# jjjkkyz/NU-NeRF

Measured on AMD Instinct MI355X. Metric: train rays/sec, higher is better.
Workload: dtype f32

## Files before the change

nu_nerf_amd/csrc/gemm_tn.hip:

```cpp
#include "gemm_epi.h"

__device__ unsigned long long nu_dbg_clk[2];

#define NU_TN_BATCH_MAX 16
struct NuGemmTNBatch {
    NuGemmTN p[NU_TN_BATCH_MAX];
    int blk0[NU_TN_BATCH_MAX + 1];
    int n, pad_;
};
static __device__ __forceinline__ int tn_batch_decode(const NuGemmTNBatch& b, int tile_edge, int& bx, int& split) {
    int pi = 0;
    for (int i = 1; i < b.n; ++i) pi = ((int)blockIdx.x >= b.blk0[i]) ? i : pi;
    const int tiles = ((b.p[pi].N1 + tile_edge - 1) / tile_edge) * ((b.p[pi].N2 + tile_edge - 1) / tile_edge);
    const int local = (int)blockIdx.x - b.blk0[pi];
    split = local / tiles;
    bx = local - split * tiles;
    return pi;
}

template <bool BIG, int PREC>
static __device__ __forceinline__ void tn_body(const NuGemmTN& g, const int bx, const int split, const int grp) {
    constexpr bool BF16 = PREC == 1;
    constexpr bool SPLIT = PREC == 2;
    constexpr int kPlane = 128 * NT_LDSH;
    __shared__ __attribute__((aligned(16))) float smem[SPLIT ? 1 : 2][SPLIT ? 3 * kPlane : 128 * NT_LDS];
    __bf16* const hA = reinterpret_cast<__bf16*>(&smem[0][0]);
    __bf16* const hB = hA + (SPLIT ? 3 : 1) * kPlane;

    const int tid = threadIdx.x;
    const int lane = tid & 63;
    const int wid = tid >> 6;
    const int wr = wid >> 1, wc = wid & 1;
    const int t2 = (g.N2 + 127) / 128;
    const int n1t = bx / t2, n2t = bx - n1t * t2;
    const int n1_0 = n1t * 128, n2_0 = n2t * 128;
    const int N1p = ((g.N1 + 127) / 128) * 128, N2p = t2 * 128;

    int rows_per = (g.P + g.S - 1) / g.S;
    rows_per = ((rows_per + TBK - 1) / TBK) * TBK;
    const int p_begin = split * rows_per;
    int p_end = p_begin + rows_per;
    p_end = p_end < g.P ? p_end : g.P;
    const int ntile = p_end > p_begin ? (p_end - p_begin + TBK - 1) / TBK : 0;
    const int npair = g.A1 ? 2 : 1;
    const int total = ntile * npair;

    const int c = tid & 127;
    const int kg = tid >> 7;
    const bool do_bias = (g.bias_slab != nullptr) && (n2t == 0);

    f32x16 acc[2][2];
#pragma unroll
    for (int i = 0; i < 2; ++i)
// ... 131 lines not shown
                acc[0][0] = __builtin_amdgcn_mfma_f32_32x32x16_bf16(a0, b0, acc[0][0], 0, 0, 0);
                acc[0][1] = __builtin_amdgcn_mfma_f32_32x32x16_bf16(a0, b1, acc[0][1], 0, 0, 0);
                acc[1][0] = __builtin_amdgcn_mfma_f32_32x32x16_bf16(a1, b0, acc[1][0], 0, 0, 0);
                acc[1][1] = __builtin_amdgcn_mfma_f32_32x32x16_bf16(a1, b1, acc[1][1], 0, 0, 0);
            }
        } else {
#pragma unroll
            for (int kk = 0; kk < 4; ++kk) {
                const float* As = &smem[0][0];
                const float* Bs = As + 128 * NT_LDS;
                const f32x4 a0 = *reinterpret_cast<const f32x4*>(&As[a_off + kk * 8]);
                const f32x4 a1 = *reinterpret_cast<const f32x4*>(&As[a_off + 32 * NT_LDS + kk * 8]);
                const f32x4 b0 = *reinterpret_cast<const f32x4*>(&Bs[b_off + kk * 8]);
                const f32x4 b1 = *reinterpret_cast<const f32x4*>(&Bs[b_off + 32 * NT_LDS + kk * 8]);
#pragma unroll
                for (int e = 0; e < 4; ++e) {
                    if (v00) acc[0][0] = __builtin_amdgcn_mfma_f32_32x32x2f32(a0[e], b0[e], acc[0][0], 0, 0, 0);
                    if (v01) acc[0][1] = __builtin_amdgcn_mfma_f32_32x32x2f32(a0[e], b1[e], acc[0][1], 0, 0, 0);
                    if (v10) acc[1][0] = __builtin_amdgcn_mfma_f32_32x32x2f32(a1[e], b0[e], acc[1][0], 0, 0, 0);
                    if (v11) acc[1][1] = __builtin_amdgcn_mfma_f32_32x32x2f32(a1[e], b1[e], acc[1][1], 0, 0, 0);
                }
            }
        }
        __syncthreads();
        if (t + 1 < total) {
            store_tile();
            __syncthreads();
        }
    }

    float* __restrict__ slab = g.slab + (long long)grp * g.sSlab + (long long)split * N1p * N2p;
#pragma unroll
    for (int tm = 0; tm < 2; ++tm)
#pragma unroll
        for (int tn = 0; tn < 2; ++tn) {
            const int col = n2_0 + wc * 64 + tn * 32 + li;
#pragma unroll
            for (int r = 0; r < 16; ++r) {
                const int row = n1_0 + wr * 64 + tm * 32 + (r & 3) + 8 * (r >> 2) + 4 * lh;
                slab[(long long)row * N2p + col] = acc[tm][tn][r];
            }
        }

    if (do_bias) {
        float* red = &smem[0][0];
        red[kg * 128 + c] = bs;
        __syncthreads();
        if (tid < 128) g.bias_slab[(long long)grp * g.sBiasSlab + (long long)split * N1p + n1_0 + tid] = red[tid] + red[128 + tid];
    }
}

template <bool BIG, int PREC>
__global__ __launch_bounds__(256, 2) void gemm_tn_kernel(NuGemmTN g) { tn_body<BIG, PREC>(g, blockIdx.x, blockIdx.y, blockIdx.z); }
template <bool BIG>
__global__ __launch_bounds__(256, 2) void gemm_tnb_kernel(NuGemmTNBatch b) {
    int bx, split;
    const int pi = tn_batch_decode(b, 128, bx, split);
    tn_body<BIG, 0>(b.p[pi], bx, split, 0);
}

#define TN16_ROWB 320
typedef short s16x4 __attribute__((ext_vector_type(4)));
typedef short s16x8 __attribute__((ext_vector_type(8)));

static __device__ __forceinline__ bf16x8 tn16_frag(const char* p) {
    const s16x4 lo = __builtin_amdgcn_ds_read_tr16_b64_v4i16((__attribute__((address_space(3))) s16x4*)(p));
    const s16x4 hi = __builtin_amdgcn_ds_read_tr16_b64_v4i16((__attribute__((address_space(3))) s16x4*)(p + 4 * TN16_ROWB));
    return __builtin_bit_cast(bf16x8, (s16x8)__builtin_shufflevector(lo, hi, 0, 1, 2, 3, 4, 5, 6, 7));
}

__global__ __launch_bounds__(256, 3) void gemm_tn16_kernel(NuGemmTN g) {
    __shared__ __attribute__((aligned(16))) char smem[2 * TBK * TN16_ROWB];
    char* const sA = smem;
    char* const sB = smem + TBK * TN16_ROWB;

    const int tid = threadIdx.x;
    const int lane = tid & 63;
    const int wid = tid >> 6;
    const int wr = wid >> 1, wc = wid & 1;
    const int t2 = (g.N2 + 127) / 128;
    const int n1t = blockIdx.x / t2, n2t = blockIdx.x - n1t * t2;
    const int split = blockIdx.y;
    const int n1_0 = n1t * 128, n2_0 = n2t * 128;
    const int grp = blockIdx.z;
    const int N1p = ((g.N1 + 127) / 128) * 128, N2p = t2 * 128;

    int rows_per = (g.P + g.S - 1) / g.S;
    rows_per = ((rows_per + TBK - 1) / TBK) * TBK;
    const int p_begin = split * rows_per;
    int p_end = p_begin + rows_per;
    p_end = p_end < g.P ? p_end : g.P;
    const int ntile = p_end > p_begin ? (p_end - p_begin + TBK - 1) / TBK : 0;
    const int npair = g.A1 ? 2 : 1;
    const int total = ntile * npair;

    const int cg = tid & 15;
    const int rr = tid >> 4;
    const bool do_bias = (g.bias_slab != nullptr) && (n2t == 0);

    f32x16 acc[2][2];
#pragma unroll
    for (int i = 0; i < 2; ++i)
#pragma unroll
        for (int j = 0; j < 2; ++j)
#pragma unroll
            for (int r = 0; r < 16; ++r) acc[i][j][r] = 0.0f;

    uint4 ra[2][2], rb[2][2];
    int nvalid = 0;
    bool pend_pair0 = true, pa16 = false, pb16 = false;
    float bs[8] = {0.f, 0.f, 0.f, 0.f, 0.f, 0.f, 0.f, 0.f};
    auto load_tile = [&](int t) {
// ... 229 lines not shown
    const int li = lane & 31, lh = lane >> 5;
    const int g4 = lane >> 4, tq = (lane & 15) >> 2, tc = lane & 3;
    const int a_off = (8 * (g4 >> 1) + tq) * TN16B_ROWB + (wr * 64 + 16 * (g4 & 1) + 4 * tc) * 2;
    const int b_off = (8 * (g4 >> 1) + tq) * TN16B_ROWB + (wc * 128 + 16 * (g4 & 1) + 4 * tc) * 2;
    for (int t = 0; t < total; ++t) {
        if (t + 1 < total) load_tile(t + 1);
#pragma unroll
        for (int ks = 0; ks < 2; ++ks) {
            const bf16x8 a0 = tn16b_frag(sA + a_off + ks * 16 * TN16B_ROWB);
            const bf16x8 a1 = tn16b_frag(sA + a_off + ks * 16 * TN16B_ROWB + 64);
            bf16x8 b[4];
#pragma unroll
            for (int tn = 0; tn < 4; ++tn) b[tn] = tn16b_frag(sB + b_off + ks * 16 * TN16B_ROWB + 64 * tn);
#pragma unroll
            for (int tn = 0; tn < 4; ++tn) {
                acc[0][tn] = __builtin_amdgcn_mfma_f32_32x32x16_bf16(a0, b[tn], acc[0][tn], 0, 0, 0);
                acc[1][tn] = __builtin_amdgcn_mfma_f32_32x32x16_bf16(a1, b[tn], acc[1][tn], 0, 0, 0);
            }
        }
        __syncthreads();
        if (t + 1 < total) {
            store_tile();
            __syncthreads();
        }
    }

    float* __restrict__ slab = g.slab + (long long)grp * g.sSlab + (long long)split * N1p * N2p;
#pragma unroll
    for (int tm = 0; tm < 2; ++tm)
#pragma unroll
        for (int tn = 0; tn < 4; ++tn) {
            const int col = n2_0 + wc * 128 + tn * 32 + li;
#pragma unroll
            for (int r = 0; r < 16; ++r) {
                const int row = n1_0 + wr * 64 + tm * 32 + (r & 3) + 8 * (r >> 2) + 4 * lh;
                slab[(long long)row * N2p + col] = acc[tm][tn][r];
            }
        }

    if (do_bias) {
        float* red = reinterpret_cast<float*>(smem);
#pragma unroll
        for (int e = 0; e < 8; ++e) red[rr * 256 + 8 * cg + e] = bs[e];
        __syncthreads();
        if (tid < 256) {
            float sum = 0.f;
#pragma unroll
            for (int r = 0; r < 16; ++r) sum += red[r * 256 + tid];
            g.bias_slab[(long long)grp * g.sBiasSlab + (long long)split * N1p + n1_0 + tid] = sum;
        }
    }
}


template <bool BIG>
static __device__ __forceinline__ void tn2_body(const NuGemmTN& g, const int bx, const int split, const int grp) {
    constexpr int T = 256;
    __shared__ __attribute__((aligned(16))) float smem[2][2][T * NT_LDS];
    const int tid = threadIdx.x;
    const int lane = tid & 63;
    const int wid = tid >> 6;
    const int wr = wid >> 1, wc = wid & 1;
    const int t2 = (g.N2 + T - 1) / T;
    const int n1t = bx / t2, n2t = bx - n1t * t2;
    const int n1_0 = n1t * T, n2_0 = n2t * T;
    const int N1p = ((g.N1 + 127) / 128) * 128, N2p = ((g.N2 + 127) / 128) * 128;

    int rows_per = (g.P + g.S - 1) / g.S;
    rows_per = ((rows_per + TBK - 1) / TBK) * TBK;
    const int p_begin = split * rows_per;
    int p_end = p_begin + rows_per;
    p_end = p_end < g.P ? p_end : g.P;
    const int ntile = p_end > p_begin ? (p_end - p_begin + TBK - 1) / TBK : 0;
    const int npair = g.A1 ? 2 : 1;
    const int total = ntile * npair;

    const int c = tid & (T - 1);
    const int kg = tid / T;
    const bool do_bias = (g.bias_slab != nullptr) && (n2t == 0);

    f32x16 acc[2][4];
#pragma unroll
    for (int i = 0; i < 2; ++i)
#pragma unroll
        for (int j = 0; j < 4; ++j)
#pragma unroll
            for (int r = 0; r < 16; ++r) acc[i][j][r] = 0.0f;

    f32x4 ra4[4], rb4[4];
    int nvalid = 16;
    bool pend_pair0 = true;
    float bs = 0.f;
    const char* __restrict__ ldA = nullptr;
    const char* __restrict__ ldB = nullptr;
    int ld_lda = 0, ld_ldb = 0, ld_ca = 0, ld_cb = 0, ld_pbase = 0, ld_pbase_u = 0;
    int nvalid_ld = 16;
    bool pair0_ld = true;
    auto load_begin = [&](int t) {
        const int pair = t >= ntile ? 1 : 0;
        const int kt = t - pair * ntile;
        ldA = (const char*)(pair ? g.A1 + (long long)grp * g.sA1 : g.A0 + (long long)grp * g.sA0);
        ldB = (const char*)(pair ? g.B1 + (long long)grp * g.sB1 : g.B0 + (long long)grp * g.sB0);
        ld_lda = pair ? g.lda1 : g.lda0;
        ld_ldb = pair ? g.ldb1 : g.ldb0;
        ld_ca = n1_0 + c; ld_cb = n2_0 + c;
        ld_ca = ld_ca < ld_lda ? ld_ca : ld_lda - 1;
        ld_cb = ld_cb < ld_ldb ? ld_cb : ld_ldb - 1;
        ld_pbase = p_begin + kt * TBK + kg * 16;
        ld_pbase_u = p_begin + kt * TBK;
        nvalid_ld = p_end - ld_pbase;
        pair0_ld = pair == 0;
    };
    auto load_piece = [&](int i, int e0, int e1) {
#pragma unroll
        for (int e = e0; e < e1; ++e) {
            int pr = ld_pbase + 4 * i + e;
            pr = pr < p_end ? pr : p_end - 1;
            if (BIG) {
                ra4[i][e] = reinterpret_cast<const float*>(ldA)[(long long)pr * ld_lda + ld_ca];
                rb4[i][e] = reinterpret_cast<const float*>(ldB)[(long long)pr * ld_ldb + ld_cb];
            } else {
                const unsigned oa = ((unsigned)pr * (unsigned)ld_lda + (unsigned)ld_ca) * 4u;
                const unsigned ob = ((unsigned)pr * (unsigned)ld_ldb + (unsigned)ld_cb) * 4u;
                ra4[i][e] = *reinterpret_cast<const float*>(ldA + oa);
                rb4[i][e] = *reinterpret_cast<const float*>(ldB + ob);
            }
        }
    };
    auto store_piece = [&](int st, int i) {
#pragma unroll
        for (int e = 0; e < 4; ++e) {
            const bool ok = 4 * i + e < nvalid;
            ra4[i][e] = ok ? ra4[i][e] : 0.f;
            rb4[i][e] = ok ? rb4[i][e] : 0.f;
        }
        if (do_bias && pend_pair0) bs += (ra4[i][0] + ra4[i][1]) + (ra4[i][2] + ra4[i][3]);
        *reinterpret_cast<f32x4*>(&smem[st][0][c * NT_LDS + kg * 16 + 4 * i]) = ra4[i];
        *reinterpret_cast<f32x4*>(&smem[st][1][c * NT_LDS + kg * 16 + 4 * i]) = rb4[i];
    };
    auto load_tile = [&](int t) {
        load_begin(t);
#pragma unroll
        for (int i = 0; i < 4; ++i) load_piece(i, 0, 4);
        nvalid = nvalid_ld; pend_pair0 = pair0_ld;
    };
    auto store_tile = [&](int st) {
#pragma unroll
        for (int i = 0; i < 4; ++i) store_piece(st, i);
    };

    if (total > 0) {
        load_tile(0);
        store_tile(0);
        if (total > 1) load_tile(1);
    }
    __syncthreads();

    const int li = lane & 31, lh = lane >> 5;
    const int a_off = (wr * 64 + li) * NT_LDS + 4 * lh;
    const int b_off = (wc * 128 + li) * NT_LDS + 4 * lh;
    struct FragT { f32x4 a[2]; f32x4 b[4]; };
    FragT F0, F1;
    const int kg_u = __builtin_amdgcn_readfirstlane(kg);
    const char* rpA = nullptr;
    const char* rpB = nullptr;
    int prA = 0, prB = 0;
    auto ld_rows_begin = [&]() {
        int pr = ld_pbase_u + kg_u * 16;
        pr = pr < p_end ? pr : p_end - 1;
        prA = prB = pr;
        rpA = ldA + (long long)pr * ld_lda * 4;
        rpB = ldB + (long long)pr * ld_ldb * 4;
    };
    auto ld_one = [&](bool isA, int i, int e) {
        if (isA) {
            ra4[i][e] = *reinterpret_cast<const float*>(rpA + (unsigned)ld_ca * 4u);
            const bool more = prA + 1 < p_end;
            rpA += more ? (long long)ld_lda * 4 : 0;
            prA += more ? 1 : 0;
        } else {
            rb4[i][e] = *reinterpret_cast<const float*>(rpB + (unsigned)ld_cb * 4u);
            const bool more = prB + 1 < p_end;
            rpB += more ? (long long)ld_ldb * 4 : 0;
            prB += more ? 1 : 0;
        }
    };
    auto st_zero = [&](bool isA, int i) {
#pragma unroll
        for (int e = 0; e < 4; ++e) {
            if (isA) ra4[i][e] = (4 * i + e < nvalid) ? ra4[i][e] : 0.f;
            else rb4[i][e] = (4 * i + e < nvalid) ? rb4[i][e] : 0.f;
        }
    };
    bool bias_on = false;
    auto st_write = [&](bool isA, int st, int i) {
        if (isA) {
            const float rs = (ra4[i][0] + ra4[i][1]) + (ra4[i][2] + ra4[i][3]);
            bs += bias_on ? rs : 0.f;
            *reinterpret_cast<f32x4*>(&smem[st][0][c * NT_LDS + kg * 16 + 4 * i]) = ra4[i];
        } else {
            *reinterpret_cast<f32x4*>(&smem[st][1][c * NT_LDS + kg * 16 + 4 * i]) = rb4[i];
        }
    };
    int cur = 0;
    if (total > 0) {
#pragma unroll
        for (int i = 0; i < 2; ++i) F0.a[i] = *reinterpret_cast<const f32x4*>(&smem[0][0][a_off + 32 * i * NT_LDS]);
#pragma unroll
        for (int j = 0; j < 4; ++j) F0.b[j] = *reinterpret_cast<const f32x4*>(&smem[0][1][b_off + 32 * j * NT_LDS]);
    }
#define TN_PIN __builtin_amdgcn_sched_barrier(0);
#define TN_M(F, e, i, j) acc[i][j] = __builtin_amdgcn_mfma_f32_32x32x2f32(F.a[i][e], F.b[j][e], acc[i][j], 0, 0, 0); TN_PIN
#define TN_SLOT(F, e, ...) TN_SLOT_(F, e, __VA_ARGS__)
#define TN_SLOT_(F, e, X0, X1, X2, X3, X4, X5, X6)                                                   \
    TN_M(F, e, 0, 0) X0; TN_PIN TN_M(F, e, 0, 1) X1; TN_PIN TN_M(F, e, 0, 2) X2; TN_PIN TN_M(F, e, 0, 3) X3; TN_PIN     \
    TN_M(F, e, 1, 0) X4; TN_PIN TN_M(F, e, 1, 1) X5; TN_PIN TN_M(F, e, 1, 2) X6; TN_PIN TN_M(F, e, 1, 3)
#define TN_RDA(F, ST, kk, i) F.a[i] = *reinterpret_cast<const f32x4*>(&smem[ST][0][a_off + 32 * (i) * NT_LDS + (kk) * 8])
#define TN_RDB(F, ST, kk, j) F.b[j] = *reinterpret_cast<const f32x4*>(&smem[ST][1][b_off + 32 * (j) * NT_LDS + (kk) * 8])
#define TN_READS(F, ST, kk) TN_RDA(F, ST, kk, 0), TN_RDA(F, ST, kk, 1), TN_RDB(F, ST, kk, 0), TN_RDB(F, ST, kk, 1), TN_RDB(F, ST, kk, 2), TN_RDB(F, ST, kk, 3), (void)0
#define TN_LD2(i, e) ld_one(true, i, e), ld_one(false, i, e), ld_one(true, i, (e) + 1), ld_one(false, i, (e) + 1), (void)0, (void)0, (void)0
#define TN_ST(i) st_zero(true, i), st_write(true, cur ^ 1, i), st_zero(false, i), st_write(false, cur ^ 1, i), (void)0, (void)0, (void)0
    for (int t = 0; t < total; ++t) {
        bias_on = do_bias && pend_pair0 && t + 1 < total;
        load_begin(t + 2 < total ? t + 2 : total - 1);
        ld_rows_begin();
        TN_SLOT(F0, 0, TN_ST(0))
        TN_SLOT(F0, 1, TN_LD2(0, 0))
        TN_SLOT(F0, 2, TN_LD2(0, 2))
        TN_SLOT(F0, 3, TN_READS(F1, cur, 1))
        TN_SLOT(F1, 0, TN_ST(1))
        TN_SLOT(F1, 1, TN_LD2(1, 0))
        TN_SLOT(F1, 2, TN_LD2(1, 2))
        TN_SLOT(F1, 3, TN_READS(F0, cur, 2))
        TN_SLOT(F0, 0, TN_ST(2))
        TN_SLOT(F0, 1, TN_ST(3))
        TN_SLOT(F0, 2, TN_LD2(2, 0))
        TN_SLOT(F0, 3, TN_READS(F1, cur, 3))
        __syncthreads();
        TN_SLOT(F1, 0, TN_LD2(2, 2))
        TN_SLOT(F1, 1, TN_LD2(3, 0))
        TN_SLOT(F1, 2, TN_LD2(3, 2))
        TN_SLOT(F1, 3, TN_READS(F0, cur ^ 1, 0))
        nvalid = nvalid_ld; pend_pair0 = pair0_ld;
        cur ^= 1;
    }
#undef TN_PIN
#undef TN_M
#undef TN_SLOT
#undef TN_SLOT_
#undef TN_RDA
#undef TN_RDB
#undef TN_READS
#undef TN_LD2
#undef TN_ST

    float* __restrict__ slab = g.slab + (long long)grp * g.sSlab + (long long)split * N1p * N2p;
#pragma unroll
    for (int tm = 0; tm < 2; ++tm)
#pragma unroll
        for (int tn = 0; tn < 4; ++tn) {
            const int col = n2_0 + wc * 128 + tn * 32 + li;
#pragma unroll
            for (int r = 0; r < 16; ++r) {
                const int row = n1_0 + wr * 64 + tm * 32 + (r & 3) + 8 * (r >> 2) + 4 * lh;
                slab[(long long)row * N2p + col] = acc[tm][tn][r];
            }
        }
    if (do_bias) {
        float* red = &smem[0][0][0];
        red[kg * T + c] = bs;
        __syncthreads();
        if (tid < T) g.bias_slab[(long long)grp * g.sBiasSlab + (long long)split * N1p + n1_0 + tid] = red[tid] + red[T + tid];
    }
}

template <bool BIG>
__global__ __launch_bounds__(512, 2) void gemm_tn2_kernel(NuGemmTN g) { tn2_body<BIG>(g, blockIdx.x, blockIdx.y, blockIdx.z); }
template <bool BIG>
__global__ __launch_bounds__(512, 2) void gemm_tn2b_kernel(NuGemmTNBatch b) {
    int bx, split;
    const int pi = tn_batch_decode(b, 256, bx, split);
    tn2_body<BIG>(b.p[pi], bx, split, 0);
}

static bool nu_tn_big_tile(int N1, int N2, int groups, int prec, int S) {
    if ((prec & 3) == 2 || (N1 % 256) != 0 || (N2 % 256) != 0) return false;
    return (long long)(N1 / 256) * (N2 / 256) * (groups > 0 ? groups : 1) * S >= 192;
}
extern "C" int nu_wgrad_pick_split(int P, int N1, int N2, int groups, int prec) {
    if (groups < 1) groups = 1;
    const int rows_min = P <= 8192 ? 128 : 256;
    const int cap = (P + rows_min - 1) / rows_min > 0 ? (P + rows_min - 1) / rows_min : 1;
    if ((N1 % 256) == 0 && (N2 % 256) == 0) {
        int S = 256 / ((N1 / 256) * (N2 / 256) * groups);
        if (S < 1) S = 1;
        if (S > cap) S = cap;
        if (nu_tn_big_tile(N1, N2, groups, prec, S)) return S;
    }
    int S = 512 / (nu_cdiv(N1, 128) * nu_cdiv(N2, 128) * groups);
    if (S < 1) S = 1;
    if (S > cap) S = cap;
    return S;
}

int nu_gemm_tn_launch(const NuGemmTN& g, hipStream_t stream) {
    if (g.N1 <= 0 || g.N2 <= 0 || g.S <= 0) return NU_ERR_ARG;
    if ((g.lda0 & 3) || (g.ldb0 & 3) || (g.A1 && ((g.lda1 & 3) || (g.ldb1 & 3)))) return NU_ERR_ARG;
    const int prec = g.bf16 & 3;
    if (prec == 3 || ((g.bf16 & ~3) && prec != 1)) return NU_ERR_ARG;
    const bool big_tile = nu_tn_big_tile(g.N1, g.N2, g.groups, g.bf16, g.S);
    const long long max_ld = (g.lda0 > g.ldb0 ? g.lda0 : g.ldb0) > (g.A1 ? (g.lda1 > g.ldb1 ? g.lda1 : g.ldb1) : 0)
                                 ? (g.lda0 > g.ldb0 ? g.lda0 : g.ldb0) : (g.lda1 > g.ldb1 ? g.lda1 : g.ldb1);
    const bool big = (long long)g.P * max_ld * 4 >= (1LL << 32);
    if (prec == 0 && big_tile) {
        dim3 grid2((g.N1 / 256) * (g.N2 / 256), g.S, g.groups > 0 ? g.groups : 1);
        if (big) hipLaunchKernelGGL((gemm_tn2_kernel<true>), grid2, dim3(512), 0, stream, g);
        else hipLaunchKernelGGL((gemm_tn2_kernel<false>), grid2, dim3(512), 0, stream, g);
        return nu_launch_status();
    }
    dim3 grid(nu_cdiv(g.N1, 128) * nu_cdiv(g.N2, 128), g.S, g.groups > 0 ? g.groups : 1), block(256);
    if (prec == 1) {
        auto ok = [](const float* p, int ld, bool h) { return p == nullptr || ((((uintptr_t)p) & 15) == 0 && ld >= 8 && (!h || (ld & 7) == 0)); };
        const bool vec = ok(g.A0, g.lda0, g.bf16 & NU_TN_A0_16) && ok(g.B0, g.ldb0, g.bf16 & NU_TN_B0_16) &&
                         ok(g.A1, g.lda1, g.bf16 & NU_TN_A1_16) && ok(g.B1, g.ldb1, g.bf16 & NU_TN_B1_16) &&
                         ((g.sA0 | g.sB0 | g.sA1 | g.sB1) & 7) == 0;
        if (vec) {
            if (big_tile) {
                dim3 grid2((g.N1 / 256) * (g.N2 / 256), g.S, g.groups > 0 ? g.groups : 1);
                hipLaunchKernelGGL(gemm_tn16x256_kernel, grid2, dim3(512), 0, stream, g);
            } else {
                hipLaunchKernelGGL(gemm_tn16_kernel, grid, block, 0, stream, g);
            }
            return nu_launch_status();
        }
    }
    if (big) {
        if (prec == 2) hipLaunchKernelGGL((gemm_tn_kernel<true, 2>), grid, block, 0, stream, g);
        else if (prec == 1) hipLaunchKernelGGL((gemm_tn_kernel<true, 1>), grid, block, 0, stream, g);
        else hipLaunchKernelGGL((gemm_tn_kernel<true, 0>), grid, block, 0, stream, g);
    } else {
        if (prec == 2) hipLaunchKernelGGL((gemm_tn_kernel<false, 2>), grid, block, 0, stream, g);
        else if (prec == 1) hipLaunchKernelGGL((gemm_tn_kernel<false, 1>), grid, block, 0, stream, g);
        else hipLaunchKernelGGL((gemm_tn_kernel<false, 0>), grid, block, 0, stream, g);
    }
    return nu_launch_status();
}

struct NuReduceBatch {
    NuReduceDesc d[NU_REDUCE_MAX];
    int n;
};

__global__ __launch_bounds__(256) void slab_reduce_batched_kernel(NuReduceBatch b) {
    __shared__ float red[256];
    int di = 0;
    for (int i = 1; i < b.n; ++i) di = ((int)blockIdx.x >= b.d[i].blk_begin) ? i : di;
    const float* __restrict__ slab = b.d[di].slab;
    float* __restrict__ out = b.d[di].out;
    const int S = b.d[di].S, N1 = b.d[di].N1, N2 = b.d[di].N2, rs = b.d[di].rs, G = b.d[di].G;
    const long long ss = b.d[di].ss;
    const int opb = 256 / G;
    const int o = threadIdx.x % opb, g = threadIdx.x / opb;
    const int idx = ((int)blockIdx.x - b.d[di].blk_begin) * opb + o;
    const bool live = idx < N1 * N2;
    float v = 0.f;
    int n1 = 0, n2 = 0;
    if (live) {
        n1 = idx / N2;
        n2 = idx - n1 * N2;
        const float* p = slab + (long long)n1 * rs + n2;
        float s0 = 0.f, s1 = 0.f, s2 = 0.f, s3 = 0.f;
        int s = g;
        for (; s + 3 * G < S; s += 4 * G) {
// ... 202 lines not shown
        float* bias_slab = w.db ? slab + slab_per * g.groups : nullptr;
        ws += (nu_wgrad_workspace_bytes(g.N1, g.N2, g.S, g.groups) + 255) / 256 * 64;
        for (int z = 0; z < g.groups; ++z) {
            NuGemmTN& q = b.p[np];
            q = g;
            q.groups = 1;
            q.A0 = g.A0 + z * g.sA0; q.B0 = g.B0 + z * g.sB0;
            q.A1 = g.A1 ? g.A1 + z * g.sA1 : nullptr; q.B1 = g.B1 ? g.B1 + z * g.sB1 : nullptr;
            q.slab = slab + z * slab_per; q.bias_slab = bias_slab ? bias_slab + z * bias_per : nullptr;
            q.sSlab = 0; q.sBiasSlab = 0;
            b.blk0[np++] = blocks;
            blocks += nu_cdiv(g.N1, edge) * nu_cdiv(g.N2, edge) * g.S;
            rc = nu_reduce_push(c->descs, &c->ndesc, c->cap, q.slab, g.S, g.N1, g.N2, N2p, (long long)N1p * N2p, w.dW + z * w.sW, w.ldw, 1.0f, 0);
            if (rc == NU_OK && w.db)
                rc = nu_reduce_push(c->descs, &c->ndesc, c->cap, q.bias_slab, g.S, g.N1, 1, 1, N1p, w.db + z * w.sDb, 1, 1.0f, 0);
            if (rc != NU_OK) return rc;
        }
        flops += w.flops; abytes += w.bytes;
    }
    b.blk0[np] = blocks;
    b.n = np; b.pad_ = 0;
    nu_ctx_ev_begin(c, stream);
    if (klass == 2) hipLaunchKernelGGL((gemm_tn2b_kernel<false>), dim3(blocks), dim3(512), 0, stream, b);
    else hipLaunchKernelGGL((gemm_tnb_kernel<false>), dim3(blocks), dim3(256), 0, stream, b);
    rc = nu_launch_status();
    nu_ctx_ev_end(c, stream, 1.0, flops, abytes);
    return rc;
}

static int wgrad_launch_single(NuOpCtx* c, NuWgradItem& w, hipStream_t stream) {
    NuGemmTN& g = w.g;
    g.S = nu_wgrad_pick_split(g.P, g.N1, g.N2, g.groups, g.bf16 & 3);
    float* ws;
    long long nb;
    int rc = nu_ctx_take(c, nu_wgrad_workspace_bytes(g.N1, g.N2, g.S, g.groups), 2 * g.groups, stream, &ws, &nb);
    if (rc != NU_OK) return rc;
    nu_ctx_ev_begin(c, stream);
    rc = nu_wgrad_enqueue(&g, w.dW, w.ldw, w.sW, w.db, w.sDb, ws, nb, c->descs, &c->ndesc, c->cap, stream);
    nu_ctx_ev_end(c, stream, 1.0, w.flops, w.bytes);
    return rc;
}

extern "C" int nu_wgrad_flush(NuOpCtx* c, hipStream_t stream) {
    const int n = c->npend;
    if (n <= 0 || c->pend == nullptr) return NU_OK;
    NuWgradItem* it = c->pend;
    c->npend = 0;
    int klass[NU_WGRAD_QUEUE_MAX];
    if (n > NU_WGRAD_QUEUE_MAX) return NU_ERR_ARG;
    int pmax = 0;
    for (int i = 0; i < n; ++i) {
        NuGemmTN& g = it[i].g;
        if (g.groups < 1) g.groups = 1;
        klass[i] = ((g.bf16 & 3) == 0 && (g.bf16 & ~3) == 0 && !tn_item_big(g) && g.groups <= NU_TN_BATCH_MAX) ? 1 : 0;
        if (klass[i] && g.P > pmax) pmax = g.P;
    }
    const int rows_min = pmax <= 8192 ? 128 : 256;
    auto plan = [&](int k, int edge, int target) -> long long {
        long long work = 0;
        for (int i = 0; i < n; ++i)
            if (klass[i] == k) work += (long long)it[i].g.P * nu_cdiv(it[i].g.N1, edge) * nu_cdiv(it[i].g.N2, edge) * it[i].g.groups;
        if (work == 0) return 0;
        long long rows = nu_cdivl(work, target);
        rows = rows < rows_min ? rows_min : rows;
        rows = nu_cdivl(rows, TBK) * TBK;
        while (true) {
            long long wgs = 0;
            for (int i = 0; i < n; ++i)
                if (klass[i] == k) wgs += nu_cdivl(it[i].g.P, rows) * nu_cdiv(it[i].g.N1, edge) * nu_cdiv(it[i].g.N2, edge) * it[i].g.groups;
            if (wgs <= target || rows >= (1LL << 30)) { for (int i = 0; i < n; ++i) if (klass[i] == k) it[i].g.S = (int)nu_cdivl(it[i].g.P, rows); return wgs; }
            rows += TBK;
        }
    };
    for (int i = 0; i < n; ++i)
        if (klass[i] == 1 && (it[i].g.N1 % 256) == 0 && (it[i].g.N2 % 256) == 0) klass[i] = 2;
    if (plan(2, 256, 256) < 192)
        for (int i = 0; i < n; ++i) if (klass[i] == 2) klass[i] = 1;
    plan(1, 128, 1024);
    for (int i = 0; i < n; ++i)
        if (klass[i] == 0) { const int rc = wgrad_launch_single(c, it[i], stream); if (rc != NU_OK) return rc; }
    for (int k = 2; k >= 1; --k) {
        int idx[NU_WGRAD_QUEUE_MAX], m = 0, nprob = 0;
        long long bytes = 0;
        for (int i = 0; i <= n; ++i) {
            const bool mine = i < n && klass[i] == k;
            long long need = 0;
            if (mine) need = (nu_wgrad_workspace_bytes(it[i].g.N1, it[i].g.N2, it[i].g.S, it[i].g.groups) + 255) / 256 * 256;
            const bool full = mine && m > 0 && (nprob + it[i].g.groups > NU_TN_BATCH_MAX || bytes + need > c->arena_floats * 4);
            if ((i == n || full) && m > 0) {
                const int rc = wgrad_launch_batch(c, it, idx, m, k, stream);
                if (rc != NU_OK) return rc;
                m = 0; nprob = 0; bytes = 0;
            }
            if (mine) { idx[m++] = i; nprob += it[i].g.groups; bytes += need; }
        }
    }
    return NU_OK;
}

extern "C" int nu_wgrad_defer(NuOpCtx* c, const NuGemmTN* g, float* dW, int ldw, long long sW, float* db, long long sDb, double flops,
                              double bytes, hipStream_t stream) {
    if (g->P <= 0) return NU_OK;
    NuWgradItem w;
    w.g = *g; w.dW = dW; w.ldw = ldw; w.pad_ = 0; w.sW = sW; w.db = db; w.sDb = sDb; w.flops = flops; w.bytes = bytes;
    if (w.g.groups < 1) w.g.groups = 1;
    if (c->pend == nullptr || c->pend_cap <= 0) return wgrad_launch_single(c, w, stream);
    if (c->npend >= c->pend_cap || c->npend >= NU_WGRAD_QUEUE_MAX) {
// ... 33 lines not shown
```

Before: 99590.

## Rewrite fp32 TN wgrad GEMM with row-major LDS tiles and vectorized loads

Replaces the tn2 body with a templated tnr_body (T=128 or 256). It stores operands row-major in LDS and loads 16-byte vectors from global memory instead of scalar column loads. A compile-time schedule interleaves LDS reads, global loads, stores and bias sums between single-k MFMA steps, and small edge tiles use fewer MFMAs. The 128-tile batched kernel and the single-launch fp32 path now route aligned inputs through this body. This is meant to cut global load count and LDS traffic, but it needs alignment checks and adds code size and register pressure.

```diff
diff --git a/nu_nerf_amd/csrc/gemm_tn.hip b/nu_nerf_amd/csrc/gemm_tn.hip
--- a/nu_nerf_amd/csrc/gemm_tn.hip
+++ b/nu_nerf_amd/csrc/gemm_tn.hip
@@ -1,4 +1,6 @@
 #include "gemm_epi.h"
+#include <type_traits>
+#include <utility>
 
 __device__ unsigned long long nu_dbg_clk[2];
 
@@ -236,12 +238,6 @@
 
 template <bool BIG, int PREC>
 __global__ __launch_bounds__(256, 2) void gemm_tn_kernel(NuGemmTN g) { tn_body<BIG, PREC>(g, blockIdx.x, blockIdx.y, blockIdx.z); }
-template <bool BIG>
-__global__ __launch_bounds__(256, 2) void gemm_tnb_kernel(NuGemmTNBatch b) {
-    int bx, split;
-    const int pi = tn_batch_decode(b, 128, bx, split);
-    tn_body<BIG, 0>(b.p[pi], bx, split, 0);
-}
 
 #define TN16_ROWB 320
 typedef short s16x4 __attribute__((ext_vector_type(4)));
@@ -577,15 +573,31 @@
     }
 }
 
-
-template <bool BIG>
-static __device__ __forceinline__ void tn2_body(const NuGemmTN& g, const int bx, const int split, const int grp) {
-    constexpr int T = 256;
-    __shared__ __attribute__((aligned(16))) float smem[2][2][T * NT_LDS];
+template <class F, int... I>
+static __device__ __forceinline__ void tn_static_for_(F&& f, std::integer_sequence<int, I...>) { (f(std::integral_constant<int, I>{}), ...); }
+template <int N, class F>
+static __device__ __forceinline__ void tn_static_for(F&& f) { tn_static_for_(f, std::make_integer_sequence<int, N>{}); }
+
+template <int T, bool BIAS>
+struct TnrSched {
+    static constexpr bool active(int s, int k) {
+        return k == 0 ? (BIAS && s <= 14) : k == 1 ? (BIAS && s == 14) : k == 2 ? true : k == 3 ? true : k == 4 ? T == 256 :
+               k == 5 ? s < 8 : k == 6 ? (s >= 1 && s <= 8) : (s == 14 || (BIAS && (s == 4 || s == 8 || s == 12 || s == 15)));
+    }
+    static constexpr int rank(int s, int k) { int n = 0; for (int i = 0; i < k; ++i) n += active(s, i) ? 1 : 0; return n; }
+    static constexpr int gap(int s, int k, int nm) { return rank(s, k) * nm / rank(s, 8); }
+};
+
+template <bool BIG, int T>
+static __device__ __forceinline__ void tnr_body(const NuGemmTN& g, const int bx, const int split, const int grp) {
+    constexpr int RS = T + 32;
+    constexpr int NB = T / 64;
+    constexpr int CG = T / 4;
+    constexpr int OPW = TBK * RS;
+    __shared__ __attribute__((aligned(16))) float smem[4 * OPW];
     const int tid = threadIdx.x;
     const int lane = tid & 63;
     const int wid = tid >> 6;
-    const int wr = wid >> 1, wc = wid & 1;
     const int t2 = (g.N2 + T - 1) / T;
     const int n1t = bx / t2, n2t = bx - n1t * t2;
     const int n1_0 = n1t * T, n2_0 = n2t * T;
@@ -600,199 +612,177 @@
     const int npair = g.A1 ? 2 : 1;
     const int total = ntile * npair;
 
-    const int c = tid & (T - 1);
+    const int cg = tid % CG;
+    const int r0 = tid / CG;
+    const int c = tid % T;
     const int kg = tid / T;
     const bool do_bias = (g.bias_slab != nullptr) && (n2t == 0);
 
-    f32x16 acc[2][4];
+    f32x16 acc[2][NB];
 #pragma unroll
     for (int i = 0; i < 2; ++i)
 #pragma unroll
-        for (int j = 0; j < 4; ++j)
+        for (int j = 0; j < NB; ++j)
 #pragma unroll
             for (int r = 0; r < 16; ++r) acc[i][j][r] = 0.0f;
 
-    f32x4 ra4[4], rb4[4];
-    int nvalid = 16;
-    bool pend_pair0 = true;
-    float bs = 0.f;
+    f32x4 ra[4], rb[4];
+    int nvalid = 0, nvalid_ld = 0;
     const char* __restrict__ ldA = nullptr;
     const char* __restrict__ ldB = nullptr;
-    int ld_lda = 0, ld_ldb = 0, ld_ca = 0, ld_cb = 0, ld_pbase = 0, ld_pbase_u = 0;
-    int nvalid_ld = 16;
-    bool pair0_ld = true;
-    auto load_begin = [&](int t) {
+    int ld_lda = 0, ld_ldb = 0, ld_ca = 0, ld_cb = 0, ld_pbase = 0;
+    const char* const pA0 = (const char*)(g.A0 + (long long)grp * g.sA0);
+    const char* const pB0 = (const char*)(g.B0 + (long long)grp * g.sB0);
+    const char* const pA1 = (const char*)(g.A1 + (long long)grp * g.sA1);
+    const char* const pB1 = (const char*)(g.B1 + (long long)grp * g.sB1);
+    const int lda0 = g.lda0, ldb0 = g.ldb0, lda1 = g.lda1, ldb1 = g.ldb1;
+    auto load_begin = [&](int t) __attribute__((always_inline)) {
         const int pair = t >= ntile ? 1 : 0;
         const int kt = t - pair * ntile;
-        ldA = (const char*)(pair ? g.A1 + (long long)grp * g.sA1 : g.A0 + (long long)grp * g.sA0);
-        ldB = (const char*)(pair ? g.B1 + (long long)grp * g.sB1 : g.B0 + (long long)grp * g.sB0);
-        ld_lda = pair ? g.lda1 : g.lda0;
-        ld_ldb = pair ? g.ldb1 : g.ldb0;
-        ld_ca = n1_0 + c; ld_cb = n2_0 + c;
-        ld_ca = ld_ca < ld_lda ? ld_ca : ld_lda - 1;
-        ld_cb = ld_cb < ld_ldb ? ld_cb : ld_ldb - 1;
-        ld_pbase = p_begin + kt * TBK + kg * 16;
-        ld_pbase_u = p_begin + kt * TBK;
+        ldA = pair ? pA1 : pA0;
+        ldB = pair ? pB1 : pB0;
+        ld_lda = pair ? lda1 : lda0;
+        ld_ldb = pair ? ldb1 : ldb0;
+        ld_ca = n1_0 + 4 * cg; ld_cb = n2_0 + 4 * cg;
+        ld_ca = ld_ca <= ld_lda - 4 ? ld_ca : ld_lda - 4;
+        ld_cb = ld_cb <= ld_ldb - 4 ? ld_cb : ld_ldb - 4;
+        ld_pbase = p_begin + kt * TBK;
         nvalid_ld = p_end - ld_pbase;
-        pair0_ld = pair == 0;
     };
-    auto load_piece = [&](int i, int e0, int e1) {
-#pragma unroll
-        for (int e = e0; e < e1; ++e) {
-            int pr = ld_pbase + 4 * i + e;
-            pr = pr < p_end ? pr : p_end - 1;
-            if (BIG) {
-                ra4[i][e] = reinterpret_cast<const float*>(ldA)[(long long)pr * ld_lda + ld_ca];
-                rb4[i][e] = reinterpret_cast<const float*>(ldB)[(long long)pr * ld_ldb + ld_cb];
-            } else {
-                const unsigned oa = ((unsigned)pr * (unsigned)ld_lda + (unsigned)ld_ca) * 4u;
-                const unsigned ob = ((unsigned)pr * (unsigned)ld_ldb + (unsigned)ld_cb) * 4u;
-                ra4[i][e] = *reinterpret_cast<const float*>(ldA + oa);
-                rb4[i][e] = *reinterpret_cast<const float*>(ldB + ob);
-            }
-        }
+    auto ld_one = [&](bool isA, int j) __attribute__((always_inline)) {
+        int pr = ld_pbase + r0 + 8 * j;
+        pr = pr < p_end ? pr : p_end - 1;
+        const char* base = isA ? ldA : ldB;
+        const int ld = isA ? ld_lda : ld_ldb, col = isA ? ld_ca : ld_cb;
+        f32x4 v;
+        if (BIG) v = *reinterpret_cast<const f32x4*>(base + ((long long)pr * ld + col) * 4);
+        else v = *reinterpret_cast<const f32x4*>(base + ((unsigned)pr * (unsigned)ld + (unsigned)col) * 4u);
+        if (isA) ra[j] = v; else rb[j] = v;
     };
-    auto store_piece = [&](int st, int i) {
-#pragma unroll
-        for (int e = 0; e < 4; ++e) {
-            const bool ok = 4 * i + e < nvalid;
-            ra4[i][e] = ok ? ra4[i][e] : 0.f;
-            rb4[i][e] = ok ? rb4[i][e] : 0.f;
-        }
-        if (do_bias && pend_pair0) bs += (ra4[i][0] + ra4[i][1]) + (ra4[i][2] + ra4[i][3]);
-        *reinterpret_cast<f32x4*>(&smem[st][0][c * NT_LDS + kg * 16 + 4 * i]) = ra4[i];
-        *reinterpret_cast<f32x4*>(&smem[st][1][c * NT_LDS + kg * 16 + 4 * i]) = rb4[i];
+    auto st_one = [&](bool isA, int st, int j) __attribute__((always_inline)) {
+        const bool ok = r0 + 8 * j < nvalid;
+        const f32x4 z = {0.f, 0.f, 0.f, 0.f};
+        const f32x4 v = isA ? ra[j] : rb[j];
+        *reinterpret_cast<f32x4*>(&smem[(2 * st + (isA ? 0 : 1)) * OPW + (r0 + 8 * j) * RS + 4 * cg]) = ok ? v : z;
     };
-    auto load_tile = [&](int t) {
-        load_begin(t);
-#pragma unroll
-        for (int i = 0; i < 4; ++i) load_piece(i, 0, 4);
-        nvalid = nvalid_ld; pend_pair0 = pair0_ld;
+
+    if (total > 0) {
+        load_begin(0);
+#pragma unroll
+        for (int j = 0; j < 4; ++j) { ld_one(true, j); ld_one(false, j); }
+        nvalid = nvalid_ld;
+#pragma unroll
+        for (int j = 0; j < 4; ++j) { st_one(true, 0, j); st_one(false, 0, j); }
+        if (total > 1) {
+            load_begin(1);
+#pragma unroll
+            for (int j = 0; j < 4; ++j) { ld_one(true, j); ld_one(false, j); }
+            nvalid = nvalid_ld;
+        }
+    }
+    __syncthreads();
+
+    const int wid_u = __builtin_amdgcn_readfirstlane(wid);
+    int arow = (wid_u >> 1) * 64, bcol = (wid_u & 1) * (T / 2), own_a = 2, own_b = NB, live_a = 2, live_b = NB;
+    if constexpr (T == 128) {
+        const int nlr = g.N1 - n1_0 >= 128 ? 4 : (g.N1 - n1_0 + 31) / 32, nlc = g.N2 - n2_0 >= 128 ? 4 : (g.N2 - n2_0 + 31) / 32;
+        if (nlc <= 2) { arow = 32 * wid_u; bcol = 0; own_a = 1; }
+        else if (nlr <= 2) { arow = 0; bcol = 32 * wid_u; own_b = 1; }
+        live_a = nlr - arow / 32; live_a = live_a < own_a ? live_a : own_a;
+        live_b = nlc - bcol / 32; live_b = live_b < own_b ? live_b : own_b;
+    }
+    const int li = lane & 31, lh = lane >> 5;
+    const int a_off = 4 * lh * RS + arow + li;
+    const int b_off = 4 * lh * RS + bcol + li;
+    const int x_off = 16 * kg * RS + c;
+    float bs = 0.f;
+    auto run = [&](auto BIAS_, auto NA_, auto NB_) __attribute__((always_inline)) {
+        constexpr bool BIAS = decltype(BIAS_)::value;
+        constexpr int NAv = decltype(NA_)::value, NBv = decltype(NB_)::value, NM = NAv * NBv;
+        using Sched = TnrSched<T, BIAS>;
+        float fa[2][2], fb[2][NB];
+        float xs[16];
+        tn_static_for<NAv>([&](auto I) { fa[0][I()] = smem[a_off + 32 * I()]; });
+        tn_static_for<NBv>([&](auto J) { fb[0][J()] = smem[OPW + b_off + 32 * J()]; });
+        int cur = 0;
+        for (int t = 0; t < total; ++t) {
+            const float* sA = smem + 2 * cur * OPW;
+            const float* sB = sA + OPW;
+            const float* nA = smem + 2 * (cur ^ 1) * OPW;
+            const float* nB = nA + OPW;
+            const bool bias_on = t < ntile;
+            load_begin(t + 2 < total ? t + 2 : total - 1);
+            tn_static_for<16>([&](auto S) {
+                constexpr int s = decltype(S)::value;
+                constexpr int rown = s < 15 ? 8 * ((s + 1) >> 2) + ((s + 1) & 3) : 0;
+                tn_static_for<NM>([&](auto M) {
+                    constexpr int m = decltype(M)::value, i = m / NBv, j = m % NBv;
+                    acc[i][j] = __builtin_amdgcn_mfma_f32_32x32x2f32(fa[s & 1][i], fb[s & 1][j], acc[i][j], 0, 0, 0);
+                    __builtin_amdgcn_sched_barrier(0);
+                    tn_static_for<8>([&](auto K) {
+                        constexpr int k = decltype(K)::value;
+                        if constexpr (Sched::active(s, k) && Sched::gap(s, k, NM) == m) {
+                            if constexpr (k == 0) xs[s] = sA[x_off + s * RS];
+                            if constexpr (k == 1) xs[15] = sA[x_off + 15 * RS];
+                            if constexpr (k == 2) {
+                                const float* p = (s < 15 ? sA : nA) + a_off + rown * RS;
+                                tn_static_for<NAv>([&](auto I) { fa[(s + 1) & 1][I()] = p[32 * I()]; });
+                            }
+                            if constexpr (k == 3 || k == 4) {
+                                const float* p = (s < 15 ? sB : nB) + b_off + rown * RS;
+                                tn_static_for<2>([&](auto J) {
+                                    constexpr int jj = 2 * (k - 3) + decltype(J)::value;
+                                    if constexpr (jj < NBv) fb[(s + 1) & 1][jj] = p[32 * jj];
+                                });
+                            }
+                            if constexpr (k == 5) st_one(s < 4, cur ^ 1, s & 3);
+                            if constexpr (k == 6) ld_one(s - 1 < 4, (s - 1) & 3);
+                            if constexpr (k == 7 && s == 14) __syncthreads();
+                            if constexpr (k == 7 && s != 14) {
+                                constexpr int q = s == 15 ? 12 : s - 4;
+                                const float rs = (xs[q] + xs[q + 1]) + (xs[q + 2] + xs[q + 3]);
+                                bs += bias_on ? rs : 0.f;
+                            }
+                            __builtin_amdgcn_sched_barrier(0);
+                        }
+                    });
+                });
+            });
+            nvalid = nvalid_ld;
+            cur ^= 1;
+        }
     };
-    auto store_tile = [&](int st) {
-#pragma unroll
-        for (int i = 0; i < 4; ++i) store_piece(st, i);
-    };
-
-    if (total > 0) {
-        load_tile(0);
-        store_tile(0);
-        if (total > 1) load_tile(1);
-    }
-    __syncthreads();
-
-    const int li = lane & 31, lh = lane >> 5;
-    const int a_off = (wr * 64 + li) * NT_LDS + 4 * lh;
-    const int b_off = (wc * 128 + li) * NT_LDS + 4 * lh;
-    struct FragT { f32x4 a[2]; f32x4 b[4]; };
-    FragT F0, F1;
-    const int kg_u = __builtin_amdgcn_readfirstlane(kg);
-    const char* rpA = nullptr;
-    const char* rpB = nullptr;
-    int prA = 0, prB = 0;
-    auto ld_rows_begin = [&]() {
-        int pr = ld_pbase_u + kg_u * 16;
-        pr = pr < p_end ? pr : p_end - 1;
-        prA = prB = pr;
-        rpA = ldA + (long long)pr * ld_lda * 4;
-        rpB = ldB + (long long)pr * ld_ldb * 4;
-    };
-    auto ld_one = [&](bool isA, int i, int e) {
-        if (isA) {
-            ra4[i][e] = *reinterpret_cast<const float*>(rpA + (unsigned)ld_ca * 4u);
-            const bool more = prA + 1 < p_end;
-            rpA += more ? (long long)ld_lda * 4 : 0;
-            prA += more ? 1 : 0;
-        } else {
-            rb4[i][e] = *reinterpret_cast<const float*>(rpB + (unsigned)ld_cb * 4u);
-            const bool more = prB + 1 < p_end;
-            rpB += more ? (long long)ld_ldb * 4 : 0;
-            prB += more ? 1 : 0;
-        }
-    };
-    auto st_zero = [&](bool isA, int i) {
-#pragma unroll
-        for (int e = 0; e < 4; ++e) {
-            if (isA) ra4[i][e] = (4 * i + e < nvalid) ? ra4[i][e] : 0.f;
-            else rb4[i][e] = (4 * i + e < nvalid) ? rb4[i][e] : 0.f;
-        }
-    };
-    bool bias_on = false;
-    auto st_write = [&](bool isA, int st, int i) {
-        if (isA) {
-            const float rs = (ra4[i][0] + ra4[i][1]) + (ra4[i][2] + ra4[i][3]);
-            bs += bias_on ? rs : 0.f;
-            *reinterpret_cast<f32x4*>(&smem[st][0][c * NT_LDS + kg * 16 + 4 * i]) = ra4[i];
-        } else {
-            *reinterpret_cast<f32x4*>(&smem[st][1][c * NT_LDS + kg * 16 + 4 * i]) = rb4[i];
-        }
-    };
-    int cur = 0;
-    if (total > 0) {
-#pragma unroll
-        for (int i = 0; i < 2; ++i) F0.a[i] = *reinterpret_cast<const f32x4*>(&smem[0][0][a_off + 32 * i * NT_LDS]);
-#pragma unroll
-        for (int j = 0; j < 4; ++j) F0.b[j] = *reinterpret_cast<const f32x4*>(&smem[0][1][b_off + 32 * j * NT_LDS]);
-    }
-#define TN_PIN __builtin_amdgcn_sched_barrier(0);
-#define TN_M(F, e, i, j) acc[i][j] = __builtin_amdgcn_mfma_f32_32x32x2f32(F.a[i][e], F.b[j][e], acc[i][j], 0, 0, 0); TN_PIN
-#define TN_SLOT(F, e, ...) TN_SLOT_(F, e, __VA_ARGS__)
-#define TN_SLOT_(F, e, X0, X1, X2, X3, X4, X5, X6)                                                   \
-    TN_M(F, e, 0, 0) X0; TN_PIN TN_M(F, e, 0, 1) X1; TN_PIN TN_M(F, e, 0, 2) X2; TN_PIN TN_M(F, e, 0, 3) X3; TN_PIN     \
-    TN_M(F, e, 1, 0) X4; TN_PIN TN_M(F, e, 1, 1) X5; TN_PIN TN_M(F, e, 1, 2) X6; TN_PIN TN_M(F, e, 1, 3)
-#define TN_RDA(F, ST, kk, i) F.a[i] = *reinterpret_cast<const f32x4*>(&smem[ST][0][a_off + 32 * (i) * NT_LDS + (kk) * 8])
-#define TN_RDB(F, ST, kk, j) F.b[j] = *reinterpret_cast<const f32x4*>(&smem[ST][1][b_off + 32 * (j) * NT_LDS + (kk) * 8])
-#define TN_READS(F, ST, kk) TN_RDA(F, ST, kk, 0), TN_RDA(F, ST, kk, 1), TN_RDB(F, ST, kk, 0), TN_RDB(F, ST, kk, 1), TN_RDB(F, ST, kk, 2), TN_RDB(F, ST, kk, 3), (void)0
-#define TN_LD2(i, e) ld_one(true, i, e), ld_one(false, i, e), ld_one(true, i, (e) + 1), ld_one(false, i, (e) + 1), (void)0, (void)0, (void)0
-#define TN_ST(i) st_zero(true, i), st_write(true, cur ^ 1, i), st_zero(false, i), st_write(false, cur ^ 1, i), (void)0, (void)0, (void)0
-    for (int t = 0; t < total; ++t) {
-        bias_on = do_bias && pend_pair0 && t + 1 < total;
-        load_begin(t + 2 < total ? t + 2 : total - 1);
-        ld_rows_begin();
-        TN_SLOT(F0, 0, TN_ST(0))
-        TN_SLOT(F0, 1, TN_LD2(0, 0))
-        TN_SLOT(F0, 2, TN_LD2(0, 2))
-        TN_SLOT(F0, 3, TN_READS(F1, cur, 1))
-        TN_SLOT(F1, 0, TN_ST(1))
-        TN_SLOT(F1, 1, TN_LD2(1, 0))
-        TN_SLOT(F1, 2, TN_LD2(1, 2))
-        TN_SLOT(F1, 3, TN_READS(F0, cur, 2))
-        TN_SLOT(F0, 0, TN_ST(2))
-        TN_SLOT(F0, 1, TN_ST(3))
-        TN_SLOT(F0, 2, TN_LD2(2, 0))
-        TN_SLOT(F0, 3, TN_READS(F1, cur, 3))
-        __syncthreads();
-        TN_SLOT(F1, 0, TN_LD2(2, 2))
-        TN_SLOT(F1, 1, TN_LD2(3, 0))
-        TN_SLOT(F1, 2, TN_LD2(3, 2))
-        TN_SLOT(F1, 3, TN_READS(F0, cur ^ 1, 0))
-        nvalid = nvalid_ld; pend_pair0 = pair0_ld;
-        cur ^= 1;
-    }
-#undef TN_PIN
-#undef TN_M
-#undef TN_SLOT
-#undef TN_SLOT_
-#undef TN_RDA
-#undef TN_RDB
-#undef TN_READS
-#undef TN_LD2
-#undef TN_ST
+    using std::integral_constant;
+    if constexpr (T == 256) {
+        if (do_bias) run(integral_constant<bool, true>{}, integral_constant<int, 2>{}, integral_constant<int, NB>{});
+        else run(integral_constant<bool, false>{}, integral_constant<int, 2>{}, integral_constant<int, NB>{});
+    } else {
+        const bool vr1 = live_a > 1, vc1 = live_b > 1;
+        auto run_b = [&](auto BIAS_) __attribute__((always_inline)) {
+            if (vr1 && vc1) run(BIAS_, integral_constant<int, 2>{}, integral_constant<int, 2>{});
+            else if (vr1) run(BIAS_, integral_constant<int, 2>{}, integral_constant<int, 1>{});
+            else if (vc1) run(BIAS_, integral_constant<int, 1>{}, integral_constant<int, 2>{});
+            else run(BIAS_, integral_constant<int, 1>{}, integral_constant<int, 1>{});
+        };
+        if (do_bias) run_b(integral_constant<bool, true>{});
+        else run_b(integral_constant<bool, false>{});
+    }
 
     float* __restrict__ slab = g.slab + (long long)grp * g.sSlab + (long long)split * N1p * N2p;
 #pragma unroll
     for (int tm = 0; tm < 2; ++tm)
 #pragma unroll
-        for (int tn = 0; tn < 4; ++tn) {
-            const int col = n2_0 + wc * 128 + tn * 32 + li;
+        for (int tn = 0; tn < NB; ++tn) {
+            if (tm >= own_a || tn >= own_b) continue;
+            const int col = n2_0 + bcol + tn * 32 + li;
 #pragma unroll
             for (int r = 0; r < 16; ++r) {
-                const int row = n1_0 + wr * 64 + tm * 32 + (r & 3) + 8 * (r >> 2) + 4 * lh;
+                const int row = n1_0 + arow + tm * 32 + (r & 3) + 8 * (r >> 2) + 4 * lh;
                 slab[(long long)row * N2p + col] = acc[tm][tn][r];
             }
         }
     if (do_bias) {
-        float* red = &smem[0][0][0];
+        float* red = smem;
         red[kg * T + c] = bs;
         __syncthreads();
         if (tid < T) g.bias_slab[(long long)grp * g.sBiasSlab + (long long)split * N1p + n1_0 + tid] = red[tid] + red[T + tid];
@@ -800,12 +790,18 @@
 }
 
 template <bool BIG>
-__global__ __launch_bounds__(512, 2) void gemm_tn2_kernel(NuGemmTN g) { tn2_body<BIG>(g, blockIdx.x, blockIdx.y, blockIdx.z); }
+__global__ __launch_bounds__(256, 2) void gemm_tnb_kernel(NuGemmTNBatch b) {
+    int bx, split;
+    const int pi = tn_batch_decode(b, 128, bx, split);
+    tnr_body<BIG, 128>(b.p[pi], bx, split, 0);
+}
+template <bool BIG>
+__global__ __launch_bounds__(512, 2) void gemm_tn2_kernel(NuGemmTN g) { tnr_body<BIG, 256>(g, blockIdx.x, blockIdx.y, blockIdx.z); }
 template <bool BIG>
 __global__ __launch_bounds__(512, 2) void gemm_tn2b_kernel(NuGemmTNBatch b) {
     int bx, split;
     const int pi = tn_batch_decode(b, 256, bx, split);
-    tn2_body<BIG>(b.p[pi], bx, split, 0);
+    tnr_body<BIG, 256>(b.p[pi], bx, split, 0);
 }
 
 static bool nu_tn_big_tile(int N1, int N2, int groups, int prec, int S) {
@@ -828,6 +824,13 @@
     return S;
 }
 
+static bool nu_tn_aligned(const NuGemmTN& g) {
+    auto ok = [](const float* p) { return (((uintptr_t)p) & 15) == 0; };
+    const bool strides = g.groups <= 1 || ((g.sA0 | g.sB0 | (g.A1 ? (g.sA1 | g.sB1) : 0)) & 3) == 0;
+    return ok(g.A0) && ok(g.B0) && (g.A1 == nullptr || (ok(g.A1) && ok(g.B1))) && strides &&
+           !((g.lda0 | g.ldb0 | (g.A1 ? (g.lda1 | g.ldb1) : 0)) & 3);
+}
+
 int nu_gemm_tn_launch(const NuGemmTN& g, hipStream_t stream) {
     if (g.N1 <= 0 || g.N2 <= 0 || g.S <= 0) return NU_ERR_ARG;
     if ((g.lda0 & 3) || (g.ldb0 & 3) || (g.A1 && ((g.lda1 & 3) || (g.ldb1 & 3)))) return NU_ERR_ARG;
@@ -837,13 +840,34 @@
     const long long max_ld = (g.lda0 > g.ldb0 ? g.lda0 : g.ldb0) > (g.A1 ? (g.lda1 > g.ldb1 ? g.lda1 : g.ldb1) : 0)
                                  ? (g.lda0 > g.ldb0 ? g.lda0 : g.ldb0) : (g.lda1 > g.ldb1 ? g.lda1 : g.ldb1);
     const bool big = (long long)g.P * max_ld * 4 >= (1LL << 32);
-    if (prec == 0 && big_tile) {
-        dim3 grid2((g.N1 / 256) * (g.N2 / 256), g.S, g.groups > 0 ? g.groups : 1);
-        if (big) hipLaunchKernelGGL((gemm_tn2_kernel<true>), grid2, dim3(512), 0, stream, g);
-        else hipLaunchKernelGGL((gemm_tn2_kernel<false>), grid2, dim3(512), 0, stream, g);
-        return nu_launch_status();
-    }
-    dim3 grid(nu_cdiv(g.N1, 128) * nu_cdiv(g.N2, 128), g.S, g.groups > 0 ? g.groups : 1), block(256);
+    const int groups = g.groups > 0 ? g.groups : 1;
+    if (prec == 0 && nu_tn_aligned(g)) {
+        if (big_tile) {
+            dim3 grid2((g.N1 / 256) * (g.N2 / 256), g.S, groups);
+            if (big) hipLaunchKernelGGL((gemm_tn2_kernel<true>), grid2, dim3(512), 0, stream, g);
+            else hipLaunchKernelGGL((gemm_tn2_kernel<false>), grid2, dim3(512), 0, stream, g);
+            return nu_launch_status();
+        }
+        if (!big && groups <= NU_TN_BATCH_MAX) {
+            NuGemmTNBatch b;
+            const int per = nu_cdiv(g.N1, 128) * nu_cdiv(g.N2, 128) * g.S;
+            for (int z = 0; z < groups; ++z) {
+                NuGemmTN& q = b.p[z];
+                q = g;
+                q.groups = 1;
+                q.A0 = g.A0 + z * g.sA0; q.B0 = g.B0 + z * g.sB0;
+                q.A1 = g.A1 ? g.A1 + z * g.sA1 : nullptr; q.B1 = g.B1 ? g.B1 + z * g.sB1 : nullptr;
+                q.slab = g.slab + z * g.sSlab; q.bias_slab = g.bias_slab ? g.bias_slab + z * g.sBiasSlab : nullptr;
+                q.sSlab = 0; q.sBiasSlab = 0;
+                b.blk0[z] = z * per;
+            }
+            b.blk0[groups] = groups * per;
+            b.n = groups; b.pad_ = 0;
+            hipLaunchKernelGGL((gemm_tnb_kernel<false>), dim3(groups * per), dim3(256), 0, stream, b);
+            return nu_launch_status();
+        }
+    }
+    dim3 grid(nu_cdiv(g.N1, 128) * nu_cdiv(g.N2, 128), g.S, groups), block(256);
     if (prec == 1) {
         auto ok = [](const float* p, int ld, bool h) { return p == nullptr || ((((uintptr_t)p) & 15) == 0 && ld >= 8 && (!h || (ld & 7) == 0)); };
         const bool vec = ok(g.A0, g.lda0, g.bf16 & NU_TN_A0_16) && ok(g.B0, g.ldb0, g.bf16 & NU_TN_B0_16) &&
@@ -1152,7 +1176,7 @@
     for (int i = 0; i < n; ++i) {
         NuGemmTN& g = it[i].g;
         if (g.groups < 1) g.groups = 1;
-        klass[i] = ((g.bf16 & 3) == 0 && (g.bf16 & ~3) == 0 && !tn_item_big(g) && g.groups <= NU_TN_BATCH_MAX) ? 1 : 0;
+        klass[i] = ((g.bf16 & 3) == 0 && (g.bf16 & ~3) == 0 && !tn_item_big(g) && g.groups <= NU_TN_BATCH_MAX && nu_tn_aligned(g)) ? 1 : 0;
         if (klass[i] && g.P > pmax) pmax = g.P;
     }
     const int rows_min = pmax <= 8192 ? 128 : 256;
```

New measurement: 99870 (median of 6 runs). No clear change (+0.3%).
